# dluvizon/scene-aware-3d-multi-human

Measured on AMD Instinct MI355X. Metric: optimizer iterations/sec (N humans x T frames), higher is better.
Workload: dtype f32 (the two dense LBS contractions as split-16-bit MFMA operands -- three products of (hi, lo) fp16 / bf16 terms, fp32 accumulate; everything else plain fp32)

## Files before the change

### scene-aware-3d-multi-human_amd/csrc/mh_raster.hip

```cpp
#include "mh_common.h"
#include "mh_raster_p.h"
#include "mh_experiment.h"

#define RS_EMPTY 0xffffffffffffffffull
#define R_KEPS 1e-8f
#define BLUR_D 1e-4f
#define BLUR_S 2e-5f
#define SIGMA_S 1e-4f
#ifndef RB
#define RB 512
#endif
#ifndef RMINW
#define RMINW 4
#endif
#ifndef R_CAP
#define R_CAP 704
#endif
#define RT 13

__device__ __forceinline__ int r_ord(float x) { const int i = __float_as_int(x); return i ^ ((i >> 31) & 0x7fffffff); }
__device__ __forceinline__ float r_unord(int o) { return __int_as_float(o ^ ((o >> 31) & 0x7fffffff)); }
#define RS_TAG(b, m) (0x5bd1e995c0ffee00ull ^ ((unsigned long long)(b) * 0x9E3779B97F4A7C15ull) ^ (unsigned long long)(m))

__device__ __forceinline__ float r_pix_to_ndc(int i, int S1, int S2) {
// ... 913 lines not shown
    R_TMARK(6);
  }
#ifdef MH_EXPERIMENT_TIMING
  R_TIMING_FLUSH();
#else
  if (p.pairs) {
    __shared__ unsigned long long s_cnt[RW][2];
    __syncthreads();
    if (lane == 0) { s_cnt[wave][0] = n_cand; s_cnt[wave][1] = n_eval; }
    R_NEAR_FLUSH();
    __syncthreads();
    if (tid == 0) {
      unsigned long long a = 0ull, b2 = 0ull;
      for (int w = 0; w < RW; ++w) { a += s_cnt[w][0]; b2 += s_cnt[w][1]; }
      unsigned long long* slot = p.pairs + 2 + 2 * (size_t)blockIdx.x;
      slot[0] += a; slot[1] += b2;
      if (blockIdx.x == 0) p.pairs[0] += 1ull;
    }
  }
#endif
}

__device__ __forceinline__ float r_alpha(const RasterP& p, const float* nb, const unsigned long long* q, float xf, float yf) {
  float qprod = 1.f;
  for (int k = 1; k < 5; ++k) {
    const unsigned long long kk = q[k];
    if (kk == RS_EMPTY) break;
    Tri tr;
    r_load_tri_ndc(p, nb, (int)(kk & 0xffffffffu), tr);
    const float T9[9] = {tr.x[0], tr.y[0], tr.z[0], tr.x[1], tr.y[1], tr.z[1], tr.x[2], tr.y[2], tr.z[2]};
    float pz, d;
    bool inside;
    r_eval(T9, xf, yf, &pz, &inside, &d);
    const float sd = inside ? -d : d;
    qprod *= 1.f - 1.f / (1.f + expf(sd / SIGMA_S));
  }
  return 1.f - qprod;
}

__global__ __launch_bounds__(RB) void k_raster_sums(RasterP p) {
  __shared__ float sh[RB / 64];
  const int tid = threadIdx.x;
  const int H = p.H, W = p.W, P = H * W;
  const int total = p.total[0];
  for (int si = blockIdx.x; si < total; si += gridDim.x) {
    const int s = p.strip_order[si];
    const int b = p.strip_body[s], t = b / p.N, n = b % p.N;
    const int x0 = p.strip_col0[s], tw = p.strip_cols[s];
    const int sy0 = p.strip_row0[s], npx = p.strip_rows[s] * tw;
    const int wx0 = p.win[b * 4], wy0 = p.win[b * 4 + 1], ww = p.win[b * 4 + 2];
    const float* vb = p.ndc + (size_t)b * p.V * 3;
    const unsigned long long* gk = p.gkeys + (size_t)p.body_koff[b] * 5;
    const float min_z = logf(1.f + expf(p.zmin_lin[t]));
    const float max_z = min_z + 1.f + logf(1.f + expf(p.zmax_lin[t]));
    const float inv_min = 1.f / min_z, inv_max = 1.f / max_z, dspan = inv_min - inv_max;
    const float pvalid = p.p2d_valid[b];
    const uint32_t fr = p.front[b];
    float lA = 0.f, lB = 0.f, lC = 0.f, lS1 = 0.f, lS2 = 0.f, lCorr = 0.f;
    for (int i = tid; i < npx; i += RB) {
      const int yi = sy0 + i / tw, xi = x0 + i % tw;
      const size_t gp = (size_t)t * P + (size_t)yi * W + xi;
      const unsigned long long* q = gk + ((size_t)(yi - wy0) * ww + (xi - wx0)) * 5;
      const unsigned long long k0 = q[0];
      if (k0 != RS_EMPTY) {
        const float z = __uint_as_float((unsigned)(k0 >> 32));
        const float m = (z > 0.f ? 1.f : 0.f) * (float)((p.ebits[gp] >> n) & 1u) * pvalid;
        if (m != 0.f) {
          const float pred = 1.f / fmaxf(z + 0.2f, p.eps);
          const float dh = p.depths[gp];
          const float tg = dh * dspan + inv_max;
          lA += logf(fmaxf(pred, 1e-3f));
          lB += logf(fmaxf(tg, 1e-3f));
          lC += 1.f;
          if (tg >= 1e-3f) {
            lS1 += dh / tg;
            lS2 += (1.f - dh) / tg;
          }
        }
        if (p.zbuf_out) p.zbuf_out[(size_t)b * P + (size_t)yi * W + xi] = z;
      }
      if (q[1] != RS_EMPTY) {
        const float alpha = r_alpha(p, vb, q, r_pix_to_ndc(W - 1 - xi, W, H), r_pix_to_ndc(H - 1 - yi, H, W));
        const uint32_t wb = p.bits[gp];
        if ((wb & fr) == 0u) {
          const float seg = (float)((wb >> n) & 1u);
          lCorr += alpha * alpha - 2.f * alpha * seg;
        }
        if (p.alpha_out) p.alpha_out[(size_t)b * P + (size_t)yi * W + xi] = alpha;
      }
    }
    lA = r_block_sum(lA, sh); lB = r_block_sum(lB, sh); lC = r_block_sum(lC, sh);
    lS1 = r_block_sum(lS1, sh); lS2 = r_block_sum(lS2, sh); lCorr = r_block_sum(lCorr, sh);
    if (tid == 0) {
      float* o = p.partial + (size_t)s * 6;
      o[0] = lA; o[1] = lB; o[2] = lC; o[3] = lS1; o[4] = lS2; o[5] = lCorr;
    }
  }
}

__device__ __forceinline__ void r_body_sums(const RasterP& p, int b, float out[6]) {
#pragma unroll
  for (int k = 0; k < 6; ++k) out[k] = 0.f;
  const int first = p.body_first[b], ns = p.body_ns[b];
  for (int s = first; s < first + ns; ++s)
#pragma unroll
    for (int k = 0; k < 6; ++k) out[k] += p.partial[(size_t)s * 6 + k];
}

__device__ __forceinline__ void r_body_sums_wave(const RasterP& p, int b, float out[6]) {
#pragma unroll
  for (int k = 0; k < 6; ++k) out[k] = 0.f;
  const int lane = threadIdx.x & 63;
  const int first = p.body_first[b], ns = p.body_ns[b];
  for (int s0 = 0; s0 < ns; s0 += 10) {
    const int m = min(10, ns - s0);
    const float v = lane < m * 6 ? p.partial[(size_t)(first + s0) * 6 + lane] : 0.f;
    for (int s = 0; s < m; ++s)
#pragma unroll
      for (int k = 0; k < 6; ++k) out[k] += __builtin_bit_cast(float, __builtin_amdgcn_readlane(__builtin_bit_cast(int, v), s * 6 + k));
  }
}

__global__ void k_raster_body_out(RasterP p) {
  const int b = blockIdx.x * blockDim.x + threadIdx.x;
  if (b >= p.B) return;
  float S[6];
  r_body_sums(p, b, S);
  const float cnt = S[2] + 1.f;
  const float diff = S[0] / cnt - S[1] / cnt;
  p.depth_body[b] = diff * diff;
  p.sil_body[b] = p.sil_apply[b] * (p.sil_S[b] + S[5]) / (p.sil_D[b] + 1.f);
  const float gB = p.coef_depth * (-2.f) * diff / cnt;
  p.dinv[(size_t)b * 2] = gB * S[3];
  p.dinv[(size_t)b * 2 + 1] = gB * S[4];
  p.sil_corr[b] = 0.f;
}

#define RFIN 1024
__global__ __launch_bounds__(RFIN) void k_raster_finish(mh_raster_fin f) {
  __shared__ float s_g0[MH_FIN_U * RFIN], s_g1[MH_FIN_U * RFIN];
  mh_raster_finish_job<RFIN>(f, s_g0, s_g1);
}

struct RgBody {
  int t, n, x0, sy0, ww;
  const float* vb;
  float* gvb;
  const unsigned long long* gk;
  float gA, gAlphaScale, pvalid;
  bool sil_on;
  uint32_t fr;
};

template <int MODE>
__device__ __forceinline__ void rg_pixel(const RasterP& p, const RgBody& bd, const int i, float& lcorr, RgDet& dc) {
  const int H = p.H, W = p.W, P = H * W;
  const int t = bd.t, n = bd.n, x0 = bd.x0, sy0 = bd.sy0, ww = bd.ww;
  const float* vb = bd.vb;
  float* gvb = bd.gvb;
  const unsigned long long* gk = bd.gk;
  const float gA = bd.gA, gAlphaScale = bd.gAlphaScale, pvalid = bd.pvalid;
  const bool sil_on = bd.sil_on;
  const uint32_t fr = bd.fr;
  const int yi = sy0 + i / ww, xi = x0 + i % ww;
  const size_t gp = (size_t)t * P + (size_t)yi * W + xi;
  const float yf = r_pix_to_ndc(H - 1 - yi, H, W), xf = r_pix_to_ndc(W - 1 - xi, W, H);
  const unsigned long long* q = gk + (size_t)i * 5;
  const unsigned long long k0 = q[0];
  if (k0 != RS_EMPTY && gA != 0.f) {
    const float z = __uint_as_float((unsigned)(k0 >> 32));
    const float m = (z > 0.f ? 1.f : 0.f) * (float)((p.ebits[gp] >> n) & 1u) * pvalid;
    const float zc = z + 0.2f;
    if (m != 0.f && zc > p.eps && 1.f / zc > 1e-3f) {
      const float gpz = -gA * r_rcp(zc);
      Tri tr;
      r_load_tri_ndc(p, vb, (int)(k0 & 0xffffffffu), tr);
      const float area = r_edge(tr.x[2], tr.y[2], tr.x[0], tr.y[0], tr.x[1], tr.y[1]) + R_KEPS;
      const float ia = r_rcp(area);
      float w[3] = {r_edge(xf, yf, tr.x[1], tr.y[1], tr.x[2], tr.y[2]) * ia,
                    r_edge(xf, yf, tr.x[2], tr.y[2], tr.x[0], tr.y[0]) * ia,
                    r_edge(xf, yf, tr.x[0], tr.y[0], tr.x[1], tr.y[1]) * ia};
      const float c[3] = {fmaxf(w[0], 0.f), fmaxf(w[1], 0.f), fmaxf(w[2], 0.f)};
      const float craw = c[0] + c[1] + c[2];
      const float cs = fmaxf(craw, 1e-5f);
      const float ics = r_rcp(cs);
      float gwc[3], gz[3], nw[3];
      float dotn = 0.f;
#pragma unroll
      for (int k = 0; k < 3; ++k) {
        nw[k] = c[k] / cs;
        gz[k] = gpz * nw[k];
        gwc[k] = gpz * tr.z[k];
        dotn += gwc[k] * nw[k];
      }
      float gw[3];
#pragma unroll
      for (int k = 0; k < 3; ++k) {
        float gc;
        if (craw > 1e-5f) {
          float acc = 0.f;
#pragma unroll
          for (int j = 0; j < 3; ++j)
            if (j != k) acc += (tr.z[k] - tr.z[j]) * nw[j];
          gc = gpz * acc * ics;
        } else {
          gc = gwc[k] * ics;
        }
        gw[k] = w[k] > 0.f ? gc : 0.f;
      }
      (void)dotn;
      const float ge[3] = {gw[0] * ia, gw[1] * ia, gw[2] * ia};
      const float garea = -(gw[0] * w[0] + gw[1] * w[1] + gw[2] * w[2]) * ia;
      float gx[3] = {0, 0, 0}, gy[3] = {0, 0, 0};
#define EDGE_ADJ(gE, A, Bv)                                           \
  gx[A] += (gE) * (yf - tr.y[Bv]);  gy[A] += (gE) * (tr.x[Bv] - xf);  \
  gx[Bv] += (gE) * (-(yf - tr.y[A])); gy[Bv] += (gE) * (xf - tr.x[A]);
      EDGE_ADJ(ge[0], 1, 2)
      EDGE_ADJ(ge[1], 2, 0)
      EDGE_ADJ(ge[2], 0, 1)
#undef EDGE_ADJ
      gx[2] += garea * (tr.y[1] - tr.y[0]);  gy[2] += garea * (-(tr.x[1] - tr.x[0]));
      gx[0] += garea * (tr.y[2] - tr.y[1]);  gy[0] += garea * (tr.x[1] - tr.x[2]);
      gx[1] += garea * (-(tr.y[2] - tr.y[0])); gy[1] += garea * (tr.x[2] - tr.x[0]);
#pragma unroll
      for (int k = 0; k < 3; ++k) r_scatter<MODE>(p, gvb, tr, k, gx[k], gy[k], gz[k], dc);
    }
  }
  const uint32_t wb = p.bits[gp];
  if (sil_on && (wb & fr) == 0u && q[1] != RS_EMPTY) {
    Tri trs[4];
    bool have[4];
#pragma unroll
    for (int k = 0; k < 4; ++k) {
      const unsigned long long kk = q[k + 1];
      have[k] = kk != RS_EMPTY;
      if (have[k]) r_load_tri_ndc(p, vb, (int)(kk & 0xffffffffu), trs[k]);
    }
    float pk[4], sgn[4], gqx[4], gqy[4], wa[4], wb_[4];
    int ea[4], eb[4];
    float qprod = 1.f;
#pragma unroll
    for (int k = 0; k < 4; ++k) {
      pk[k] = 0.f; sgn[k] = 0.f; gqx[k] = gqy[k] = wa[k] = wb_[k] = 0.f; ea[k] = 0; eb[k] = 1;
      if (!have[k]) continue;
      const Tri& tr = trs[k];
      const float area = r_edge(tr.x[2], tr.y[2], tr.x[0], tr.y[0], tr.x[1], tr.y[1]) + R_KEPS;
      const float ia = r_rcp(area);
      const bool inside = r_edge(xf, yf, tr.x[1], tr.y[1], tr.x[2], tr.y[2]) * ia > 0.f &&
                          r_edge(xf, yf, tr.x[2], tr.y[2], tr.x[0], tr.y[0]) * ia > 0.f &&
                          r_edge(xf, yf, tr.x[0], tr.y[0], tr.x[1], tr.y[1]) * ia > 0.f;
      float t01, t02, t12;
      bool g01, g02, g12;
      const float d01 = r_seg_rcp(xf, yf, tr.x[0], tr.y[0], tr.x[1], tr.y[1], &t01, &g01);
      const float d02 = r_seg_rcp(xf, yf, tr.x[0], tr.y[0], tr.x[2], tr.y[2], &t02, &g02);
      const float d12 = r_seg_rcp(xf, yf, tr.x[1], tr.y[1], tr.x[2], tr.y[2], &t12, &g12);
      float d, tt;
      bool dg;
      int a, bb;
      if (d01 <= d02 && d01 <= d12) { d = d01; a = 0; bb = 1; tt = t01; dg = g01; }
      else if (d02 <= d01 && d02 <= d12) { d = d02; a = 0; bb = 2; tt = t02; dg = g02; }
      else { d = d12; a = 1; bb = 2; tt = t12; dg = g12; }
      const float xa_ = a == 0 ? tr.x[0] : tr.x[1], ya_ = a == 0 ? tr.y[0] : tr.y[1];
      const float xb_ = bb == 1 ? tr.x[1] : tr.x[2], yb_ = bb == 1 ? tr.y[1] : tr.y[2];
      if (dg) { gqx[k] = xb_ - xf; gqy[k] = yb_ - yf; wa[k] = 0.f; wb_[k] = 1.f; }
      else {
        gqx[k] = xa_ + tt * (xb_ - xa_) - xf;
        gqy[k] = ya_ + tt * (yb_ - ya_) - yf;
        wa[k] = 1.f - tt; wb_[k] = tt;
      }
      ea[k] = a; eb[k] = bb;
      const float sd = inside ? -d : d;
      pk[k] = r_rcp(1.f + expf(sd * (1.f / SIGMA_S)));
      sgn[k] = inside ? -1.f : 1.f;
      qprod *= 1.f - pk[k];
    }
    const float alpha = 1.f - qprod;
    const float seg = (float)((wb >> n) & 1u);
    lcorr += alpha * alpha - 2.f * alpha * seg;
    const float galpha = gAlphaScale * (alpha - seg);
    if (galpha != 0.f) {
      int eid[8];
      float egx[8], egy[8], egz[8];
#pragma unroll
      for (int k = 0; k < 4; ++k) {
        eid[2 * k] = eid[2 * k + 1] = -1;
        egx[2 * k] = egy[2 * k] = egz[2 * k] = egx[2 * k + 1] = egy[2 * k + 1] = egz[2 * k + 1] = 0.f;
        if (!have[k]) continue;
        const float gd = galpha * (-(1.f / SIGMA_S)) * pk[k] * qprod * sgn[k];
        if (gd == 0.f) continue;
        const Tri& tr = trs[k];
        const bool a0 = ea[k] == 0, b1 = eb[k] == 1;
        const int ia_ = a0 ? tr.idx[0] : tr.idx[1], ib_ = b1 ? tr.idx[1] : tr.idx[2];
        const float xa = a0 ? tr.x[0] : tr.x[1], ya = a0 ? tr.y[0] : tr.y[1], za = a0 ? tr.z[0] : tr.z[1];
        const float xb = b1 ? tr.x[1] : tr.x[2], yb = b1 ? tr.y[1] : tr.y[2], zb = b1 ? tr.z[1] : tr.z[2];
        const float gxn = gd * 2.f * gqx[k], gyn = gd * 2.f * gqy[k];
        if (wa[k] != 0.f) {
          const float rz = r_rcp(za), ux = wa[k] * gxn, uy = wa[k] * gyn;
          eid[2 * k] = ia_;
          egx[2 * k] = -p.s * rz * ux; egy[2 * k] = -p.s * rz * uy; egz[2 * k] = -((xa - p.w1) * ux + (ya - p.h1) * uy) * rz;
        }
        if (wb_[k] != 0.f) {
          const float rz = r_rcp(zb), ux = wb_[k] * gxn, uy = wb_[k] * gyn;
          eid[2 * k + 1] = ib_;
          egx[2 * k + 1] = -p.s * rz * ux; egy[2 * k + 1] = -p.s * rz * uy; egz[2 * k + 1] = -((xb - p.w1) * ux + (yb - p.h1) * uy) * rz;
        }
      }
#ifndef RG_NOMERGE
#pragma unroll
      for (int i = 1; i < 8; ++i) {
        bool merged = false;
#pragma unroll
        for (int j = 0; j < i; ++j) {
          const bool hit = !merged && eid[i] >= 0 && eid[j] == eid[i];
          egx[j] += hit ? egx[i] : 0.f;
          egy[j] += hit ? egy[i] : 0.f;
          egz[j] += hit ? egz[i] : 0.f;
          merged = merged || hit;
        }
        if (merged) eid[i] = -1;
      }
#endif
#pragma unroll
      for (int i = 0; i < 8; ++i)
        if (eid[i] >= 0) r_acc_add<MODE>(gvb, eid[i], egx[i], egy[i], egz[i], dc);
    }
  }
}

#ifndef RGB
#define RGB 1024
#endif
template <bool TAB>
__global__ __launch_bounds__(RGB) void k_raster_grads(RasterP p) {
  __shared__ float s_red[RGB / 64];
  float* gtab = rg_tab;
  const int tid = threadIdx.x;
  const int H = p.H, W = p.W, P = H * W;
  const bool use_tab = TAB;
  int* plist = (int*)(gtab + (use_tab ? p.V * 3 : 0));
  int* s_n = plist + RG_LIST;
  const int nunits = p.gunit_total[0];
  RG_TIMING_DECL();
  r_deferred_sorts<RGB>(p, (int*)gtab);
  int xb = -1, xk = 0, xend = 0;
  for (int u = blockIdx.x;;) {
    int b, piece;
    if (xk < xend) {
      b = xb; piece = xk++;
    } else if (u < nunits) {
      const unsigned long long ue = p.gunit_list[u];
      u += gridDim.x;
      b = (int)(ue >> 32); piece = (int)(ue & 0xffffffffu);
    } else if (u < nunits + p.B) {
      xb = u - nunits;
      u += gridDim.x;
      const int wx = p.win[xb * 4 + 2], wy = p.win[xb * 4 + 3];
      const int nu = (wx > 0 && wy > 0) ? (wx * wy + RG_UNIT - 1) / RG_UNIT : 0;
      xk = min(p.nu_listed[xb], nu); xend = nu;
      continue;
    } else {
      break;
    }
    const int up0 = piece * RG_UNIT;
    const int t = b / p.N, n = b % p.N;
    const int x0 = p.win[b * 4], ww = p.win[b * 4 + 2], y0 = p.win[b * 4 + 1], wh = p.win[b * 4 + 3];
    if (ww <= 0 || wh <= 0 || up0 >= ww * wh) continue;
    const int npx = min(ww * wh, up0 + RG_UNIT);
    const int sy0 = y0;
    const float* vb = p.ndc + (size_t)b * p.V * 3;
    float* gvb = p.gverts + (size_t)b * p.V * 3;
    const unsigned long long* gk = p.gkeys + (size_t)p.body_koff[b] * 5;
    float S[6];
#if RG_WAVE_SUMS
    r_body_sums_wave(p, b, S);
#else
    r_body_sums(p, b, S);
#endif
    const float cnt = S[2] + 1.f;
    const float diff = S[0] / cnt - S[1] / cnt;
    const float gA = p.coef_depth * 2.f * diff / cnt;
    const float gAlphaScale = p.coef_sil * p.sil_apply[b] * 2.f / (p.sil_D[b] + 1.f);
    const bool sil_on = p.sil_apply[b] != 0.f;
    float lcorr = 0.f;
    const float pvalid = p.p2d_valid[b];
    const uint32_t fr = p.front[b];
    RgBody bd;
    bd.t = t; bd.n = n; bd.x0 = x0; bd.sy0 = sy0; bd.ww = ww; bd.vb = vb; bd.gvb = gvb; bd.gk = gk;
    bd.gA = gA; bd.gAlphaScale = gAlphaScale; bd.pvalid = pvalid; bd.sil_on = sil_on; bd.fr = fr;
    RgDet dc;
    bool table_clear = !use_tab;
    RG_TMARK(0);
    for (int cbase = up0; cbase < npx; cbase += RG_LIST) {
    constexpr int NPT = (RG_LIST + RGB - 1) / RGB;
    unsigned long long c0[NPT], c1[NPT];
    uint32_t ceb[NPT], cbt[NPT];
    const int cend = min(cbase + RG_LIST, npx);
#pragma unroll
    for (int j = 0; j < NPT; ++j) {
      const int i = min(cbase + tid + j * RGB, cend - 1);
      const int yi = sy0 + i / ww, xi = x0 + i % ww;
      const size_t gp = (size_t)t * P + (size_t)yi * W + xi;
      const unsigned long long* q = gk + (size_t)i * 5;
      c0[j] = q[0]; c1[j] = q[1];
      ceb[j] = p.ebits[gp]; cbt[j] = p.bits[gp];
    }
    if (tid == 0) *s_n = 0;
    if (!table_clear) {
      __syncthreads();
      for (int i = tid; i < p.V * 3; i += RGB) gtab[i] = 0.f;
      table_clear = true;
    }
    __syncthreads();
    RG_TMARK(1);
#pragma unroll
    for (int j = 0; j < NPT; ++j) {
      const int i = cbase + tid + j * RGB;
      const bool dep = gA != 0.f && pvalid != 0.f && c0[j] != RS_EMPTY && ((ceb[j] >> n) & 1u);
      const bool sil = sil_on && c1[j] != RS_EMPTY && (cbt[j] & fr) == 0u;
      const bool live = i < cend && (dep || sil);
      const unsigned long long m = __ballot(live);
      if (m) {
        int base = 0;
        const int lane = tid & 63;
        if (lane == 0) base = atomicAdd(s_n, __popcll(m));
        base = __shfl(base, 0, 64);
        if (live) plist[base + __popcll(m & ((1ull << lane) - 1ull))] = i;
      }
    }
    __syncthreads();
    RG_TMARK(2);
    const int nlive = *s_n;
    for (int li_ = tid; li_ < nlive; li_ += RGB) {
      const int i = plist[li_];
      rg_pixel<TAB ? 1 : 0>(p, bd, i, lcorr, dc);
    }
    __syncthreads();
    RG_TMARK(3);
    }
    lcorr = r_block_sum(lcorr, s_red);
    if (tid == 0 && lcorr != 0.f) atomicAdd(&p.sil_corr[b], lcorr);
    if (use_tab)
      for (int i = tid; i < p.V * 3; i += RGB) {
        const float g = gtab[i];
        if (g != 0.f) atomicAdd(&gvb[i], g);
      }
    RG_TMARK(4);
  }
  RG_TIMING_FLUSH();
}

__global__ __launch_bounds__(RGB) void k_raster_grads_det(RasterP p) {
  __shared__ float s_red[RGB / 64];
  __shared__ int s_shift;
  unsigned long long* tab = (unsigned long long*)rg_tab;
  const int tid = threadIdx.x;
  const int H = p.H, W = p.W, P = H * W;
  const int VH = (p.V + 1) / 2;
  for (int b = blockIdx.x; b < p.B; b += gridDim.x) {
    const int t = b / p.N, n = b % p.N;
    const int x0 = p.win[b * 4], ww = p.win[b * 4 + 2], y0 = p.win[b * 4 + 1], wh = p.win[b * 4 + 3];
    if (ww <= 0 || wh <= 0) continue;
    const int npx = ww * wh;
    float S[6];
    r_body_sums(p, b, S);
    const float cnt = S[2] + 1.f;
    const float diff = S[0] / cnt - S[1] / cnt;
    RgBody bd;
    bd.t = t; bd.n = n; bd.x0 = x0; bd.sy0 = y0; bd.ww = ww;
    bd.vb = p.ndc + (size_t)b * p.V * 3;
    bd.gvb = p.gverts + (size_t)b * p.V * 3;
    bd.gk = p.gkeys + (size_t)p.body_koff[b] * 5;
    bd.gA = p.coef_depth * 2.f * diff / cnt;
    bd.gAlphaScale = p.coef_sil * p.sil_apply[b] * 2.f / (p.sil_D[b] + 1.f);
    bd.sil_on = p.sil_apply[b] != 0.f;
    bd.pvalid = p.p2d_valid[b];
    bd.fr = p.front[b];
    RgDet dc;
    dc.umax = 0.f; dc.shift = 0;
    float lcorr = 0.f;
    for (int pass = 0; pass < 3; ++pass) {
      dc.pass = pass;
      dc.v0 = pass == 2 ? VH : 0;
      dc.v1 = pass == 1 ? VH : p.V;
      __syncthreads();
      if (pass > 0) {
        dc.shift = s_shift;
        for (int i = tid; i < VH * 3; i += RGB) tab[i] = 0ull;
        __syncthreads();
      }
      float lc = 0.f;
      for (int i = tid; i < npx; i += RGB) {
        const int yi = y0 + i / ww, xi = x0 + i % ww;
        const size_t gp = (size_t)t * P + (size_t)yi * W + xi;
        const unsigned long long* q = bd.gk + (size_t)i * 5;
        const bool dep = bd.gA != 0.f && bd.pvalid != 0.f && q[0] != RS_EMPTY && ((p.ebits[gp] >> n) & 1u);
        const bool sil = bd.sil_on && q[1] != RS_EMPTY && (p.bits[gp] & bd.fr) == 0u;
        if (dep || sil) rg_pixel<2>(p, bd, i, lc, dc);
      }
      if (pass == 0) {
        lcorr = r_block_sum(lc, s_red);
        float m = dc.umax;
#pragma unroll
        for (int o = 32; o > 0; o >>= 1) m = fmaxf(m, __shfl_xor(m, o, 64));
        __syncthreads();
        if ((tid & 63) == 0) s_red[tid >> 6] = m;
        __syncthreads();
        if (tid == 0) {
          float mm = 0.f;
          for (int w = 0; w < RGB / 64; ++w) mm = fmaxf(mm, s_red[w]);
          int e = 0;
          if (mm > 0.f && mm < INFINITY) (void)frexpf(mm, &e);
          s_shift = 46 - e;
        }
      } else {
        __syncthreads();
        const int nv = (dc.v1 - dc.v0) * 3;
        float* o = bd.gvb + (size_t)dc.v0 * 3;
        for (int i = tid; i < nv; i += RGB) {
          const long long a = (long long)tab[i];
          if (a != 0) o[i] += (float)ldexp((double)a, -dc.shift);
        }
      }
    }
    if (tid == 0 && lcorr != 0.f) p.sil_corr[b] += lcorr;
  }
  __syncthreads();
  r_deferred_sorts<RGB>(p, (int*)rg_tab);
}

__global__ void k_fill(float* x, size_t n, float v) {
  for (size_t i = blockIdx.x * (size_t)blockDim.x + threadIdx.x; i < n; i += (size_t)gridDim.x * blockDim.x) x[i] = v;
}

static int g_raster_det = -1;
static bool raster_deterministic() {
  if (g_raster_det < 0) {
    const char* e = getenv("MHHIP_DETERMINISTIC");
    g_raster_det = (e && e[0] == '1') ? 1 : 0;
  }
  return g_raster_det != 0;
}
extern "C" int mh_raster_set_deterministic(int on) {
  g_raster_det = on ? 1 : 0;
  return MH_OK;
}
extern "C" int mh_raster_get_deterministic(void) { return raster_deterministic() ? 1 : 0; }

static int g_raster_margin = -1;
static int raster_sort_margin() {
  if (g_raster_margin < 0) {
    const char* e = getenv("MHHIP_RASTER_SORT_MARGIN");
    g_raster_margin = e ? atoi(e) : 1;
    if (g_raster_margin < 0 || g_raster_margin > 8) g_raster_margin = 1;
  }
  return g_raster_margin;
}
extern "C" int mh_raster_set_sort_margin(int rows) {
  MH_CHECK(rows >= 0 && rows <= 8, "margin must be 0..8 rows");
  g_raster_margin = rows;
  return MH_OK;
}
extern "C" int mh_raster_get_sort_margin(void) { return raster_sort_margin(); }
static float g_raster_defer = -1.f;
static float raster_sort_defer() {
  if (g_raster_defer < 0.f) {
    const char* e = getenv("MHHIP_RASTER_SORT_DEFER");
    g_raster_defer = e ? (float)atof(e) : 0.6f;
    if (!(g_raster_defer >= 0.f && g_raster_defer <= 1.f)) g_raster_defer = 0.6f;
  }
  return g_raster_defer;
}
static float raster_sort_soft(int margin) {
  const float hard = (float)margin - 0.02f, f = raster_sort_defer();
  return (f > 0.f && f < 1.f && margin > 0) ? fminf(f * (float)margin, hard) : hard;
}
extern "C" int mh_raster_set_sort_defer(float fraction) {
  MH_CHECK(fraction >= 0.f && fraction <= 1.f, "fraction of the margin: 0..1 (0 or 1: no deferred sorts)");
  g_raster_defer = fraction;
  return MH_OK;
}
extern "C" float mh_raster_get_sort_defer(void) { return raster_sort_defer(); }
static int g_raster_all_even = 0;
extern "C" int mh_raster_set_path(int all_even) {
  g_raster_all_even = all_even ? 1 : 0;
  return MH_OK;
}
extern "C" int mh_raster_get_path(void) { return g_raster_all_even; }

static int g_raster_winners = -1;
static int raster_winners() {
  if (g_raster_winners < 0) {
    const char* e = getenv("MHHIP_RASTER_WINNERS");
    g_raster_winners = (e && e[0] == '0') ? 0 : 1;
  }
  return g_raster_winners;
}
extern "C" int mh_raster_set_winners(int on) {
  g_raster_winners = on ? 1 : 0;
  return MH_OK;
}
extern "C" int mh_raster_get_winners(void) { return raster_winners(); }
static size_t r_prepare_lds(const RasterP& p) {
  return ((size_t)4 * (p.H + 1) + (p.F <= R_WIN_MAXF ? (size_t)(p.F + 31) / 32 : 0)) * sizeof(int);
}

static size_t r_align(size_t x) { return (x + 255) & ~(size_t)255; }
static size_t r_max_units(size_t B, int H, int W) { return B + B * (size_t)H * W / RG_UNIT + 1; }
static int r_max_strips(int B, int H, int W) {
  const int th = W <= R_CAP ? (R_CAP / W > 0 ? R_CAP / W : 1) : R_CAP / R_TILE_W;
  const int tw = W <= R_CAP ? W : R_TILE_W;
  const int per_body = ((W + tw - 1) / tw) * ((H + th - 1) / th);
  return B * (per_body > H ? per_body : H);
}

static size_t r_carve(RasterP& p, void* ws) {
  const size_t B = (size_t)p.B;
  const int V = p.V, F = p.F, H = p.H, W = p.W;
  p.max_strips = r_max_strips(p.B, H, W);
  const size_t ms = (size_t)p.max_strips;
  char* c = (char*)ws;
  p.win = (int*)c; c += r_align(B * 4 * 4);
  p.body_first = (int*)c; c += r_align(B * 4);
  p.body_ns = (int*)c; c += r_align(B * 4);
  p.strip_body = (int*)c; c += r_align(ms * 4);
  p.strip_row0 = (int*)c; c += r_align(ms * 4);
  p.strip_rows = (int*)c; c += r_align(ms * 4);
  p.strip_col0 = (int*)c; c += r_align(ms * 4);
  p.strip_cols = (int*)c; c += r_align(ms * 4);
  p.partial = (float*)c; c += r_align(ms * 6 * 4);
  p.dinv = (float*)c; c += r_align(B * 2 * 4);
  p.ndc = (float*)c; c += r_align(B * V * 3 * 4);
  p.frows = (unsigned*)c; c += r_align(B * F * 4);
  p.fsort = (unsigned*)c; c += r_align(B * F * 4);
  p.row_start = (int*)c; c += r_align(B * (size_t)(4 * (H + 1) + 1) * 4);
  p.maxh = (int*)c; c += r_align(B * 4);
  p.body_koff = (long long*)c; c += r_align(B * 8);
  p.rowb = (float*)c; c += r_align(B * V * 4);
  p.margin = raster_sort_margin();
  p.all_even = g_raster_all_even;
  p.max_units = (int)r_max_units(B, H, W);
  p.strip_cls = (int*)c; c += r_align(ms * 4);
  p.strip_order = (int*)c; c += r_align(ms * 4);
  p.gunit_list = (unsigned long long*)c; c += r_align((size_t)p.max_units * 8);
  p.stale = (int*)c; c += r_align(B * 4);
  p.ctl = (unsigned*)c; c += r_align(16);
  p.total = (int*)c; c += r_align(4);
  p.gunit_total = (int*)c; c += r_align(4);
  p.ns_listed = (int*)c; c += r_align(B * 4);
  p.nu_listed = (int*)c; c += r_align(B * 4);
  p.sort_count = (unsigned long long*)c; c += r_align(24);
// ... 41 lines not shown
  r_carve(p, nullptr);
  out[0] = (size_t)((char*)p.win - (char*)nullptr);
  out[1] = (size_t)((char*)p.body_koff - (char*)nullptr);
  out[2] = (size_t)((char*)p.gkeys - (char*)nullptr);
  return MH_OK;
}

extern "C" int mh_raster_debug_offsets2(int T, int N, int V, int F, int H, int W, size_t* out ) {
  RasterP p;
  p.B = T * N; p.N = N; p.V = V; p.F = F; p.H = H; p.W = W;
  r_carve(p, nullptr);
  out[0] = (size_t)((char*)p.kvalid - (char*)nullptr);
  out[1] = (size_t)((char*)p.wstate - (char*)nullptr);
  out[2] = (size_t)((char*)p.sort_tag - (char*)nullptr);
  return MH_OK;
}
extern "C" int mh_raster_debug_offsets(int T, int N, int V, int F, int H, int W, size_t* out ) {
  RasterP p;
  p.B = T * N; p.N = N; p.V = V; p.F = F; p.H = H; p.W = W;
  r_carve(p, nullptr);
  out[0] = (size_t)((char*)p.ndc - (char*)nullptr);
  out[1] = (size_t)((char*)p.frows - (char*)nullptr);
  out[2] = (size_t)((char*)p.fsort - (char*)nullptr);
  out[3] = (size_t)((char*)p.row_start - (char*)nullptr);
  out[4] = (size_t)((char*)p.maxh - (char*)nullptr);
  out[5] = (size_t)((char*)p.rowb - (char*)nullptr);
  return MH_OK;
}

extern "C" int mh_raster_pair_counters(int T, int N, int V, int F, int H, int W, void* ws, unsigned long long* out_host, void* stream) {
  MH_CHECK(ws && out_host, "null argument");
  MH_CHECK(T > 0 && N > 0 && V > 0 && F > 0 && H > 0 && W > 0, "empty input");
  RasterP p;
  p.B = T * N; p.N = N; p.V = V; p.F = F; p.H = H; p.W = W;
  r_carve(p, ws);
  static unsigned long long host[2 + 2 * R_STRIP_GRID];
  MH_HIP(hipMemcpyAsync(host, p.pairs, sizeof(host), hipMemcpyDeviceToHost, (hipStream_t)stream));
  MH_HIP(hipStreamSynchronize((hipStream_t)stream));
  out_host[0] = host[0]; out_host[1] = 0ull; out_host[2] = 0ull;
  R_TIMING_HOST_SPANS();
  for (int i = 0; i < R_STRIP_GRID; ++i) { out_host[1] += host[2 + 2 * i]; out_host[2] += host[3 + 2 * i]; }
  return MH_OK;
}

extern "C" int mh_raster_sort_counters(int T, int N, int V, int F, int H, int W, void* ws, unsigned long long* out_host, void* stream) {
  MH_CHECK(ws, "null argument");
  MH_CHECK(T > 0 && N > 0 && V > 0 && F > 0 && H > 0 && W > 0, "empty input");
  RasterP p;
  p.B = T * N; p.N = N; p.V = V; p.F = F; p.H = H; p.W = W;
  r_carve(p, ws);
  if (out_host) {
    MH_HIP(hipMemcpyAsync(out_host, p.sort_count, 16, hipMemcpyDeviceToHost, (hipStream_t)stream));
    MH_HIP(hipStreamSynchronize((hipStream_t)stream));
  } else {
    MH_HIP(hipMemsetAsync(p.sort_count, 0, 24, (hipStream_t)stream));
  }
  return MH_OK;
}

extern "C" int mh_raster_sort_counters3(int T, int N, int V, int F, int H, int W, void* ws, unsigned long long* out_host, void* stream) {
  MH_CHECK(ws && out_host, "null argument");
  MH_CHECK(T > 0 && N > 0 && V > 0 && F > 0 && H > 0 && W > 0, "empty input");
  RasterP p;
  p.B = T * N; p.N = N; p.V = V; p.F = F; p.H = H; p.W = W;
  r_carve(p, ws);
  MH_HIP(hipMemcpyAsync(out_host, p.sort_count, 24, hipMemcpyDeviceToHost, (hipStream_t)stream));
  MH_HIP(hipStreamSynchronize((hipStream_t)stream));
  return MH_OK;
}

static void r_calibration(RasterP& p, const float* cam_K_host) {
  const int W = p.W, H = p.H;
  const float fx = cam_K_host[0], fy = cam_K_host[4], cx = cam_K_host[2], cy = cam_K_host[5];
  if (W > H) {
    p.s = 2.f * fy / H;
    const float u = (float)W / H;
    p.w1 = u * (W - 2.f * cx) / W;
    p.h1 = (H - 2.f * cy) / H;
  } else if (H > W) {
    p.s = 2.f * fx / W;
    const float u = (float)H / W;
    p.w1 = (W - 2.f * cx) / W;
    p.h1 = u * (H - 2.f * cy) / H;
  } else {
    p.s = 2.f * (fx + fy) / (W + H);
    p.w1 = (W - 2.f * cx) / W;
    p.h1 = (H - 2.f * cy) / H;
  }
}

static int raster_terms_impl(int T, int N, int V, int F, int H, int W, const float* cam_K_host, const float* verts,
                             const int32_t* faces, const uint32_t* bits, const uint32_t* ebits, const float* depths,
                             const float* zmin_lin, const float* zmax_lin, const float* pose2d_valid,
                             const uint32_t* front, const float* sil_apply, const float* sil_D, const float* sil_S,
                             float coef_depth, float coef_sil, float eps, float* gverts, float* gzmin, float* gzmax,
                             float* depth_body, float* sil_body, void* ws, float* zbuf_out, float* alpha_out,
                             int phases, float* log_depth, float* log_sil, void* stream, int projected = 0,
                             mh_raster_fin* fin_out = nullptr) {
  MH_CHECK(cam_K_host && (verts || projected) && faces && bits && ebits && depths && zmin_lin && zmax_lin && pose2d_valid && front &&
               sil_apply && sil_D && sil_S && depth_body && sil_body && ws,
           "null argument");
  MH_CHECK(T > 0 && N > 0 && N <= 32 && V > 0 && F > 0 && H > 0 && W > 0, "empty input");
  MH_CHECK(H <= 4095 && W <= 65535 && F < (1 << 20), "sorted face entries hold 12-bit rows and 20-bit face ids");
  MH_CHECK(V < (1 << 22), "vertex offsets of the gathers are 24-bit products (3 * vertex index)");
  RasterP p;
  p.B = T * N; p.N = N; p.V = V; p.F = F; p.H = H; p.W = W;
  r_calibration(p, cam_K_host);
  p.verts = verts; p.faces = faces; p.bits = bits; p.ebits = ebits; p.depths = depths;
  p.zmin_lin = zmin_lin; p.zmax_lin = zmax_lin; p.p2d_valid = pose2d_valid; p.front = front;
  p.sil_apply = sil_apply; p.sil_D = sil_D; p.sil_S = sil_S;
  p.coef_depth = coef_depth; p.coef_sil = coef_sil; p.eps = eps;
  p.gverts = gverts; p.depth_body = depth_body; p.sil_body = sil_body;
  p.zbuf_out = zbuf_out; p.alpha_out = alpha_out;
  r_carve(p, ws);
  p.projected = projected ? 1 : 0;
  if (mh_prof_level() < 2) p.pairs = nullptr;
  hipStream_t st = (hipStream_t)stream;
  const bool do_prep = (phases & (1 | 4)) != 0, do_sel = (phases & (1 | 8)) != 0;
  if (do_prep) {
  if (zbuf_out) {
    hipLaunchKernelGGL(k_fill, dim3(1024), dim3(256), 0, st, zbuf_out, (size_t)p.B * H * W, -1.f);
    MH_LAUNCH_CHECK();
  }
  if (alpha_out) MH_HIP(hipMemsetAsync(alpha_out, 0, (size_t)p.B * H * W * sizeof(float), st));
  mh_prof_mark(MH_PROF_RASTER_PREP, 0, st);
  hipLaunchKernelGGL(k_raster_prepare, dim3(p.B), dim3(RPREP), r_prepare_lds(p), st, p);
  MH_LAUNCH_CHECK();
  if (!(phases & 128) || !gverts || zbuf_out || alpha_out) {
    hipLaunchKernelGGL(k_raster_lists, dim3(1), dim3(RLISTS), 0, st, p);
    MH_LAUNCH_CHECK();
  }
  mh_prof_mark(MH_PROF_RASTER_PREP, 1, st);
  }
  if (do_sel) {
  const int grid = R_STRIP_GRID;
  mh_prof_mark(MH_PROF_RASTER_STRIP, 0, st);
  hipLaunchKernelGGL(k_raster_strip, dim3(grid), dim3(RB), 0, st, p);
  MH_LAUNCH_CHECK();
  mh_prof_mark(MH_PROF_RASTER_STRIP, 1, st);
  if (!gverts || zbuf_out || alpha_out) {
    mh_prof_mark(MH_PROF_RASTER_SUMS, 0, st);
    hipLaunchKernelGGL(k_raster_sums, dim3(grid), dim3(RB), 0, st, p);
    MH_LAUNCH_CHECK();
    mh_prof_mark(MH_PROF_RASTER_SUMS, 1, st);
  }
  if (!gverts || zbuf_out || alpha_out) {
    hipLaunchKernelGGL(k_raster_body_out, dim3((p.B + 255) / 256), dim3(256), 0, st, p);
    MH_LAUNCH_CHECK();
  }
  }
  if (!(phases & 2)) return MH_OK;
  if (gverts) {
    const bool use_tab = V <= RG_MAXV;
    const size_t tab = (use_tab ? (size_t)V * 3 * sizeof(float) : 0) + (RG_LIST + 1) * sizeof(int);
    static unsigned char attr_set[MH_MAX_DEVICES];
    if (mh_first_on_device(attr_set))
      MH_HIP(hipFuncSetAttribute((const void*)k_raster_grads<true>, hipFuncAttributeMaxDynamicSharedMemorySize, RG_MAXV * 3 * 4 + (RG_LIST + 1) * 4));
    mh_prof_mark(MH_PROF_RASTER_GRADS, 0, st);
    const int ggrid = 256 * 6;
    RasterP pg = p;
    if (raster_deterministic()) {
      MH_CHECK(V <= RG_MAXV, "deterministic gradient scatter: model too large for the LDS table");
      static unsigned char attr_det[MH_MAX_DEVICES];
      if (mh_first_on_device(attr_det))
        MH_HIP(hipFuncSetAttribute((const void*)k_raster_grads_det, hipFuncAttributeMaxDynamicSharedMemorySize, ((RG_MAXV + 1) / 2) * 3 * 8));
      if (r_prepare_lds(p) > (size_t)((V + 1) / 2) * 3 * 8) pg.resort = nullptr;
      hipLaunchKernelGGL(k_raster_grads_det, dim3(p.B < 4096 ? p.B : 4096), dim3(RGB), (size_t)((V + 1) / 2) * 3 * 8, st, pg);
    } else {
      if (r_prepare_lds(p) > tab) pg.resort = nullptr;
      if (use_tab) hipLaunchKernelGGL(k_raster_grads<true>, dim3(ggrid), dim3(RGB), tab, st, pg);
      else hipLaunchKernelGGL(k_raster_grads<false>, dim3(ggrid), dim3(RGB), tab, st, pg);
    }
    MH_LAUNCH_CHECK();
    mh_prof_mark(MH_PROF_RASTER_GRADS, 1, st);
  }
  if (fin_out) memset(fin_out, 0, sizeof(*fin_out));
  if (gverts || (gzmin && gzmax) || log_depth || log_sil) {
    mh_raster_fin f;
    f.T = T; f.N = N; f.B = p.B; f.from_partials = (gverts && !zbuf_out && !alpha_out) ? 1 : 0;
    f.coef_depth = p.coef_depth;
    f.body_first = p.body_first; f.body_ns = p.body_ns; f.partial = p.partial; f.dinv = p.dinv;
    f.sil_apply = p.sil_apply; f.sil_D = p.sil_D; f.sil_S = p.sil_S; f.sil_corr = p.sil_corr;
    f.depth_body = p.depth_body; f.sil_body = p.sil_body;
    f.zmin_lin = zmin_lin; f.zmax_lin = zmax_lin;
    f.gzmin = (gzmin && gzmax) ? gzmin : (float*)nullptr; f.gzmax = gzmax;
    f.log_depth = log_depth; f.log_sil = log_sil;
    if (fin_out) {
      *fin_out = f;
      if (phases & 128) {
        static_assert(sizeof(RasterP) <= sizeof(fin_out->lists), "mh_raster_fin.lists too small for the parameter block");
        memcpy(fin_out->lists, &p, sizeof(RasterP));
        fin_out->has_lists = 1;
      }
    } else {
      hipLaunchKernelGGL(k_raster_finish, dim3(1), dim3(RFIN), 0, st, f);
      MH_LAUNCH_CHECK();
    }
  }
  return MH_OK;
}

extern "C" int mh_raster_terms(int T, int N, int V, int F, int H, int W, const float* cam_K_host, const float* verts,
                               const int32_t* faces, const uint32_t* bits, const uint32_t* ebits, const float* depths,
                               const float* zmin_lin, const float* zmax_lin, const float* pose2d_valid,
                               const uint32_t* front, const float* sil_apply, const float* sil_D, const float* sil_S,
                               float coef_depth, float coef_sil, float eps, float* gverts, float* gzmin, float* gzmax,
                               float* depth_body, float* sil_body, void* ws, float* zbuf_out, float* alpha_out,
                               void* stream) {
  return raster_terms_impl(T, N, V, F, H, W, cam_K_host, verts, faces, bits, ebits, depths, zmin_lin, zmax_lin, pose2d_valid, front,
                           sil_apply, sil_D, sil_S, coef_depth, coef_sil, eps, gverts, gzmin, gzmax, depth_body, sil_body, ws, zbuf_out,
                           alpha_out, 3, nullptr, nullptr, stream);
}

extern "C" int mh_raster_terms_phase(int T, int N, int V, int F, int H, int W, const float* cam_K_host, const float* verts,
                                     const int32_t* faces, const uint32_t* bits, const uint32_t* ebits, const float* depths,
                                     const float* zmin_lin, const float* zmax_lin, const float* pose2d_valid,
                                     const uint32_t* front, const float* sil_apply, const float* sil_D, const float* sil_S,
                                     float coef_depth, float coef_sil, float eps, float* gverts, float* gzmin, float* gzmax,
                                     float* depth_body, float* sil_body, void* ws, float* zbuf_out, float* alpha_out,
                                     int phases, void* stream) {
  MH_CHECK(phases >= 1 && phases <= 3, "phases: 1 = selection + values, 2 = gradients, 3 = both");
  return raster_terms_impl(T, N, V, F, H, W, cam_K_host, verts, faces, bits, ebits, depths, zmin_lin, zmax_lin, pose2d_valid, front,
                           sil_apply, sil_D, sil_S, coef_depth, coef_sil, eps, gverts, gzmin, gzmax, depth_body, sil_body, ws, zbuf_out,
                           alpha_out, phases, nullptr, nullptr, stream);
}

extern "C" int mh_raster_terms_phase_log(int T, int N, int V, int F, int H, int W, const float* cam_K_host, const float* verts,
                                         const int32_t* faces, const uint32_t* bits, const uint32_t* ebits, const float* depths,
                                         const float* zmin_lin, const float* zmax_lin, const float* pose2d_valid,
                                         const uint32_t* front, const float* sil_apply, const float* sil_D, const float* sil_S,
                                         float coef_depth, float coef_sil, float eps, float* gverts, float* gzmin, float* gzmax,
                                         float* depth_body, float* sil_body, void* ws, float* zbuf_out, float* alpha_out,
                                         int phases, float* log_depth, float* log_sil, void* stream) {
  MH_CHECK(phases >= 1 && phases <= 3, "phases: 1 = selection + values, 2 = gradients, 3 = both");
  return raster_terms_impl(T, N, V, F, H, W, cam_K_host, verts, faces, bits, ebits, depths, zmin_lin, zmax_lin, pose2d_valid, front,
                           sil_apply, sil_D, sil_S, coef_depth, coef_sil, eps, gverts, gzmin, gzmax, depth_body, sil_body, ws, zbuf_out,
                           alpha_out, phases, log_depth, log_sil, stream);
}

extern "C" int mh_raster_terms_projected(int T, int N, int V, int F, int H, int W, const float* cam_K_host, const float* verts,
                                         const int32_t* faces, const uint32_t* bits, const uint32_t* ebits, const float* depths,
                                         const float* zmin_lin, const float* zmax_lin, const float* pose2d_valid,
                                         const uint32_t* front, const float* sil_apply, const float* sil_D, const float* sil_S,
                                         float coef_depth, float coef_sil, float eps, float* gverts, float* gzmin, float* gzmax,
                                         float* depth_body, float* sil_body, void* ws, float* zbuf_out, float* alpha_out,
                                         int phases, float* log_depth, float* log_sil, int projected, void* stream) {
  MH_CHECK(phases >= 1 && (phases & ~(15 | 128)) == 0, "phases: 1 = preparation + selection + values, 2 = gradients, 4 = preparation only, 8 = selection only, 128 = work lists deferred");
  return raster_terms_impl(T, N, V, F, H, W, cam_K_host, verts, faces, bits, ebits, depths, zmin_lin, zmax_lin, pose2d_valid, front,
                           sil_apply, sil_D, sil_S, coef_depth, coef_sil, eps, gverts, gzmin, gzmax, depth_body, sil_body, ws, zbuf_out,
                           alpha_out, phases, log_depth, log_sil, stream, projected);
}

extern "C" int mh_raster_terms_deferred(int T, int N, int V, int F, int H, int W, const float* cam_K_host, const float* verts,
                                         const int32_t* faces, const uint32_t* bits, const uint32_t* ebits, const float* depths,
                                         const float* zmin_lin, const float* zmax_lin, const float* pose2d_valid,
                                         const uint32_t* front, const float* sil_apply, const float* sil_D, const float* sil_S,
                                         float coef_depth, float coef_sil, float eps, float* gverts, float* gzmin, float* gzmax,
                                         float* depth_body, float* sil_body, void* ws, float* zbuf_out, float* alpha_out,
                                         int phases, float* log_depth, float* log_sil, int projected, mh_raster_fin* fin_out, void* stream) {
  MH_CHECK(phases >= 1 && (phases & ~(15 | 128)) == 0, "phases: 1 = preparation + selection + values, 2 = gradients, 4 = preparation only, 8 = selection only, 128 = work lists deferred");
  MH_CHECK(fin_out, "null argument");
  return raster_terms_impl(T, N, V, F, H, W, cam_K_host, verts, faces, bits, ebits, depths, zmin_lin, zmax_lin, pose2d_valid, front,
                           sil_apply, sil_D, sil_S, coef_depth, coef_sil, eps, gverts, gzmin, gzmax, depth_body, sil_body, ws, zbuf_out,
                           alpha_out, phases, log_depth, log_sil, stream, projected, fin_out);
}

extern "C" int mh_raster_forward_targets(int T, int N, int V, int F, int H, int W, const float* cam_K_host, void* ws,
                                         mh_fwd_proj* out) {
  MH_CHECK(cam_K_host && ws && out, "null argument");
  MH_CHECK(T > 0 && N > 0 && V > 0 && F > 0 && H > 0 && W > 0, "empty input");
  RasterP p;
  p.B = T * N; p.N = N; p.V = V; p.F = F; p.H = H; p.W = W;
  r_calibration(p, cam_K_host);
  r_carve(p, ws);
  out->s = p.s; out->w1 = p.w1; out->h1 = p.h1;
  float range = 2.0f;
  if (H > W) range = ((float)H * range) / (float)W;
  out->rk = (float)H / range;
  out->ra = (float)H - 0.5f - 0.5f * (float)H;
  out->thr = (float)p.margin - 0.02f;
  out->thr_soft = p.soft;
  out->slack_ndc = 0.5f * 2.0f / (float)(H < W ? H : W);
  out->slack_y = 0.005f;
  if (const char* e = getenv("MHHIP_PROJ_SLACK_PX")) out->slack_ndc = (float)atof(e) * 2.0f / (float)(H < W ? H : W);
  out->ndc = p.ndc; out->rowb = p.rowb;
  out->bbox = p.fbbox; out->bbox_prev = p.fbbox_prev;
  out->lowkey = p.flowkey; out->lowkey_prev = p.flowkey_prev;
  out->moved = p.fmoved;
  out->clear = nullptr; out->clear_n = 0ull;
  return MH_OK;
}
```

Baseline: 1553.

## Split raster-grad pixel work into separate silhouette and depth item lists

Breaks the per-pixel gradient routine into separate depth and silhouette functions and compacts live pixels into two 16-bit LDS index lists, so each thread handles one kind of item and wave divergence between the two paths drops. It also clears the LDS gradient table once per block and re-zeroes entries during flush, instead of clearing the whole table per unit. The classification loop now assumes one pass per unit, which a static assert enforces. The cost is an extra ballot and atomic per wave, plus the assumption that the table is fully cleaned after each unit.

```diff
diff --git a/scene-aware-3d-multi-human_amd/csrc/mh_raster.hip b/scene-aware-3d-multi-human_amd/csrc/mh_raster.hip
--- a/scene-aware-3d-multi-human_amd/csrc/mh_raster.hip
+++ b/scene-aware-3d-multi-human_amd/csrc/mh_raster.hip
@@ -1089,20 +1089,20 @@
   uint32_t fr;
 };
 
+#define RG_PIXEL_HEAD()                                                                      \
+  const int H = p.H, W = p.W, P = H * W;                                                     \
+  const int t = bd.t, n = bd.n, x0 = bd.x0, sy0 = bd.sy0, ww = bd.ww;                        \
+  const float* vb = bd.vb;                                                                   \
+  float* gvb = bd.gvb;                                                                       \
+  const unsigned long long* gk = bd.gk;                                                      \
+  const int yi = sy0 + i / ww, xi = x0 + i % ww;                                             \
+  const size_t gp = (size_t)t * P + (size_t)yi * W + xi;                                     \
+  const float yf = r_pix_to_ndc(H - 1 - yi, H, W), xf = r_pix_to_ndc(W - 1 - xi, W, H);      \
+  const unsigned long long* q = gk + (size_t)i * 5
 template <int MODE>
-__device__ __forceinline__ void rg_pixel(const RasterP& p, const RgBody& bd, const int i, float& lcorr, RgDet& dc) {
-  const int H = p.H, W = p.W, P = H * W;
-  const int t = bd.t, n = bd.n, x0 = bd.x0, sy0 = bd.sy0, ww = bd.ww;
-  const float* vb = bd.vb;
-  float* gvb = bd.gvb;
-  const unsigned long long* gk = bd.gk;
-  const float gA = bd.gA, gAlphaScale = bd.gAlphaScale, pvalid = bd.pvalid;
-  const bool sil_on = bd.sil_on;
-  const uint32_t fr = bd.fr;
-  const int yi = sy0 + i / ww, xi = x0 + i % ww;
-  const size_t gp = (size_t)t * P + (size_t)yi * W + xi;
-  const float yf = r_pix_to_ndc(H - 1 - yi, H, W), xf = r_pix_to_ndc(W - 1 - xi, W, H);
-  const unsigned long long* q = gk + (size_t)i * 5;
+__device__ __forceinline__ void rg_pixel_depth(const RasterP& p, const RgBody& bd, const int i, RgDet& dc) {
+  RG_PIXEL_HEAD();
+  const float gA = bd.gA, pvalid = bd.pvalid;
   const unsigned long long k0 = q[0];
   if (k0 != RS_EMPTY && gA != 0.f) {
     const float z = __uint_as_float((unsigned)(k0 >> 32));
@@ -1122,13 +1122,11 @@
       const float cs = fmaxf(craw, 1e-5f);
       const float ics = r_rcp(cs);
       float gwc[3], gz[3], nw[3];
-      float dotn = 0.f;
 #pragma unroll
       for (int k = 0; k < 3; ++k) {
         nw[k] = c[k] / cs;
         gz[k] = gpz * nw[k];
         gwc[k] = gpz * tr.z[k];
-        dotn += gwc[k] * nw[k];
       }
       float gw[3];
 #pragma unroll
@@ -1145,7 +1143,6 @@
         }
         gw[k] = w[k] > 0.f ? gc : 0.f;
       }
-      (void)dotn;
       const float ge[3] = {gw[0] * ia, gw[1] * ia, gw[2] * ia};
       const float garea = -(gw[0] * w[0] + gw[1] * w[1] + gw[2] * w[2]) * ia;
       float gx[3] = {0, 0, 0}, gy[3] = {0, 0, 0};
@@ -1163,6 +1160,13 @@
       for (int k = 0; k < 3; ++k) r_scatter<MODE>(p, gvb, tr, k, gx[k], gy[k], gz[k], dc);
     }
   }
+}
+template <int MODE>
+__device__ __forceinline__ void rg_pixel_sil(const RasterP& p, const RgBody& bd, const int i, float& lcorr, RgDet& dc) {
+  RG_PIXEL_HEAD();
+  const float gAlphaScale = bd.gAlphaScale;
+  const bool sil_on = bd.sil_on;
+  const uint32_t fr = bd.fr;
   const uint32_t wb = p.bits[gp];
   if (sil_on && (wb & fr) == 0u && q[1] != RS_EMPTY) {
     Tri trs[4];
@@ -1267,6 +1271,11 @@
 #ifndef RGB
 #define RGB 1024
 #endif
+#ifndef RG_GRID
+#define RG_GRID (256 * 6)
+#endif
+static_assert(RG_LIST == RG_UNIT && RG_UNIT <= 65536, "one classification pass per unit, 16-bit item offsets");
+#define RG_ITEM_BYTES ((size_t)2 * RG_LIST * sizeof(unsigned short) + 2 * sizeof(int))
 template <bool TAB>
 __global__ __launch_bounds__(RGB) void k_raster_grads(RasterP p) {
   __shared__ float s_red[RGB / 64];
@@ -1274,11 +1283,14 @@
   const int tid = threadIdx.x;
   const int H = p.H, W = p.W, P = H * W;
   const bool use_tab = TAB;
-  int* plist = (int*)(gtab + (use_tab ? p.V * 3 : 0));
-  int* s_n = plist + RG_LIST;
+  unsigned short* slist = (unsigned short*)(gtab + (use_tab ? p.V * 3 : 0));
+  unsigned short* dlist = slist + RG_LIST;
+  int* s_n = (int*)(dlist + RG_LIST);
   const int nunits = p.gunit_total[0];
   RG_TIMING_DECL();
   r_deferred_sorts<RGB>(p, (int*)gtab);
+  if (use_tab && (int)blockIdx.x < nunits + p.B)
+    for (int i = tid; i < p.V * 3; i += RGB) gtab[i] = 0.f;
   int xb = -1, xk = 0, xend = 0;
   for (int u = blockIdx.x;;) {
     int b, piece;
@@ -1307,6 +1319,19 @@
     const float* vb = p.ndc + (size_t)b * p.V * 3;
     float* gvb = p.gverts + (size_t)b * p.V * 3;
     const unsigned long long* gk = p.gkeys + (size_t)p.body_koff[b] * 5;
+    constexpr int NPT = (RG_UNIT + RGB - 1) / RGB;
+    unsigned long long c0[NPT], c1[NPT];
+    uint32_t ceb[NPT], cbt[NPT];
+#pragma unroll
+    for (int j = 0; j < NPT; ++j) {
+      const int i = min(up0 + tid + j * RGB, npx - 1);
+      const int yi = sy0 + i / ww, xi = x0 + i % ww;
+      const size_t gp = (size_t)t * P + (size_t)yi * W + xi;
+      const unsigned long long* q = gk + (size_t)i * 5;
+      c0[j] = q[0]; c1[j] = q[1];
+      ceb[j] = p.ebits[gp]; cbt[j] = p.bits[gp];
+    }
+    if (tid < 2) s_n[tid] = 0;
     float S[6];
 #if RG_WAVE_SUMS
     r_body_sums_wave(p, b, S);
@@ -1325,61 +1350,46 @@
     bd.t = t; bd.n = n; bd.x0 = x0; bd.sy0 = sy0; bd.ww = ww; bd.vb = vb; bd.gvb = gvb; bd.gk = gk;
     bd.gA = gA; bd.gAlphaScale = gAlphaScale; bd.pvalid = pvalid; bd.sil_on = sil_on; bd.fr = fr;
     RgDet dc;
-    bool table_clear = !use_tab;
     RG_TMARK(0);
-    for (int cbase = up0; cbase < npx; cbase += RG_LIST) {
-    constexpr int NPT = (RG_LIST + RGB - 1) / RGB;
-    unsigned long long c0[NPT], c1[NPT];
-    uint32_t ceb[NPT], cbt[NPT];
-    const int cend = min(cbase + RG_LIST, npx);
-#pragma unroll
-    for (int j = 0; j < NPT; ++j) {
-      const int i = min(cbase + tid + j * RGB, cend - 1);
-      const int yi = sy0 + i / ww, xi = x0 + i % ww;
-      const size_t gp = (size_t)t * P + (size_t)yi * W + xi;
-      const unsigned long long* q = gk + (size_t)i * 5;
-      c0[j] = q[0]; c1[j] = q[1];
-      ceb[j] = p.ebits[gp]; cbt[j] = p.bits[gp];
-    }
-    if (tid == 0) *s_n = 0;
-    if (!table_clear) {
-      __syncthreads();
-      for (int i = tid; i < p.V * 3; i += RGB) gtab[i] = 0.f;
-      table_clear = true;
-    }
     __syncthreads();
     RG_TMARK(1);
 #pragma unroll
     for (int j = 0; j < NPT; ++j) {
-      const int i = cbase + tid + j * RGB;
-      const bool dep = gA != 0.f && pvalid != 0.f && c0[j] != RS_EMPTY && ((ceb[j] >> n) & 1u);
-      const bool sil = sil_on && c1[j] != RS_EMPTY && (cbt[j] & fr) == 0u;
-      const bool live = i < cend && (dep || sil);
-      const unsigned long long m = __ballot(live);
-      if (m) {
-        int base = 0;
+      const int i = up0 + tid + j * RGB;
+      const bool dep = i < npx && gA != 0.f && pvalid != 0.f && c0[j] != RS_EMPTY && ((ceb[j] >> n) & 1u);
+      const bool sil = i < npx && sil_on && c1[j] != RS_EMPTY && (cbt[j] & fr) == 0u;
+      const unsigned long long ms = __ballot(sil), md = __ballot(dep);
+      if (ms | md) {
+        int bs = 0, bdp = 0;
         const int lane = tid & 63;
-        if (lane == 0) base = atomicAdd(s_n, __popcll(m));
-        base = __shfl(base, 0, 64);
-        if (live) plist[base + __popcll(m & ((1ull << lane) - 1ull))] = i;
+        if (lane == 0) {
+          if (ms) bs = atomicAdd(s_n, __popcll(ms));
+          if (md) bdp = atomicAdd(s_n + 1, __popcll(md));
+        }
+        bs = __shfl(bs, 0, 64); bdp = __shfl(bdp, 0, 64);
+        const unsigned long long below = (1ull << lane) - 1ull;
+        if (sil) slist[bs + __popcll(ms & below)] = (unsigned short)(i - up0);
+        if (dep) dlist[bdp + __popcll(md & below)] = (unsigned short)(i - up0);
       }
     }
     __syncthreads();
     RG_TMARK(2);
-    const int nlive = *s_n;
-    for (int li_ = tid; li_ < nlive; li_ += RGB) {
-      const int i = plist[li_];
-      rg_pixel<TAB ? 1 : 0>(p, bd, i, lcorr, dc);
+    const int n_sil = s_n[0], n_items = n_sil + s_n[1];
+    for (int it = tid; it < n_items; it += RGB) {
+      if (it < n_sil) rg_pixel_sil<TAB ? 1 : 0>(p, bd, up0 + (int)slist[it], lcorr, dc);
+      else rg_pixel_depth<TAB ? 1 : 0>(p, bd, up0 + (int)dlist[it - n_sil], dc);
     }
     __syncthreads();
     RG_TMARK(3);
-    }
     lcorr = r_block_sum(lcorr, s_red);
     if (tid == 0 && lcorr != 0.f) atomicAdd(&p.sil_corr[b], lcorr);
     if (use_tab)
       for (int i = tid; i < p.V * 3; i += RGB) {
         const float g = gtab[i];
-        if (g != 0.f) atomicAdd(&gvb[i], g);
+        if (g != 0.f) {
+          gtab[i] = 0.f;
+          atomicAdd(&gvb[i], g);
+        }
       }
     RG_TMARK(4);
   }
@@ -1432,7 +1442,10 @@
         const unsigned long long* q = bd.gk + (size_t)i * 5;
         const bool dep = bd.gA != 0.f && bd.pvalid != 0.f && q[0] != RS_EMPTY && ((p.ebits[gp] >> n) & 1u);
         const bool sil = bd.sil_on && q[1] != RS_EMPTY && (p.bits[gp] & bd.fr) == 0u;
-        if (dep || sil) rg_pixel<2>(p, bd, i, lc, dc);
+        if (dep || sil) {
+          rg_pixel_depth<2>(p, bd, i, dc);
+          rg_pixel_sil<2>(p, bd, i, lc, dc);
+        }
       }
       if (pass == 0) {
         lcorr = r_block_sum(lc, s_red);
@@ -1780,12 +1793,12 @@
   if (!(phases & 2)) return MH_OK;
   if (gverts) {
     const bool use_tab = V <= RG_MAXV;
-    const size_t tab = (use_tab ? (size_t)V * 3 * sizeof(float) : 0) + (RG_LIST + 1) * sizeof(int);
+    const size_t tab = (use_tab ? (size_t)V * 3 * sizeof(float) : 0) + RG_ITEM_BYTES;
     static unsigned char attr_set[MH_MAX_DEVICES];
     if (mh_first_on_device(attr_set))
-      MH_HIP(hipFuncSetAttribute((const void*)k_raster_grads<true>, hipFuncAttributeMaxDynamicSharedMemorySize, RG_MAXV * 3 * 4 + (RG_LIST + 1) * 4));
+      MH_HIP(hipFuncSetAttribute((const void*)k_raster_grads<true>, hipFuncAttributeMaxDynamicSharedMemorySize, (int)(RG_MAXV * 3 * 4 + RG_ITEM_BYTES)));
     mh_prof_mark(MH_PROF_RASTER_GRADS, 0, st);
-    const int ggrid = 256 * 6;
+    const int ggrid = RG_GRID;
     RasterP pg = p;
     if (raster_deterministic()) {
       MH_CHECK(V <= RG_MAXV, "deterministic gradient scatter: model too large for the LDS table");
```

Result: no change. 1547 (-0.4%).
